# leggedrobotics/art_planner

Hardware: AMD Instinct MI355X
Metric: validated states/sec on 400x400@0.04m map (sample + validity check) (higher is better)
Workload: dtype f32; 1 GPU; C2: lazy_prm_star_min_update front end, 400x400@0.04m Perlin terrain (seed 1234) + 12 obstacles, YAML robot, batch sampler + validity checker; map=400x400@0.04, lanes=1

## Files before the change

art_planner_amd/context.py:

```python
from __future__ import annotations

import ctypes as C
from typing import Optional

import numpy as np

from . import _capi


def make_params(kind="yaml", **overrides) -> _capi.Params:
    L = _capi.load()
    p = _capi.Params()
    (L.artp_params_yaml if kind == "yaml" else L.artp_params_defaults)(C.byref(p))
    for k, v in overrides.items():
        setattr(p, k, v)
    return p


def _f32F(a) -> np.ndarray:
    return np.asfortranarray(a, dtype=np.float32)


class Context:

# ... 120 lines not shown

    def set_z_bounds(self, z_low, z_high):
        self._chk(self.L.artp_set_z_bounds(self.h, float(z_low), float(z_high)), "artp_set_z_bounds")
        self.z_bounds = (float(z_low), float(z_high))

    def set_r3_extent(self, max_extent):
        self._chk(self.L.artp_set_r3_extent(self.h, float(max_extent)), "artp_set_r3_extent")

    def check_motions_last_valid(self, s1, s2):
        s1 = np.ascontiguousarray(s1, np.float64).reshape(-1, 7)
        s2 = np.ascontiguousarray(s2, np.float64).reshape(-1, 7)
        n = s1.shape[0]
        valid = np.empty(n, np.uint8)
        t = np.empty(n, np.float64)
        st = np.empty((n, 7), np.float64)
        self._chk(self.L.artp_check_motions_last_valid(self.h, s1.ctypes.data, s2.ctypes.data, n, valid.ctypes.data,
                                                       t.ctypes.data, st.ctypes.data), "artp_check_motions_last_valid")
        return valid, t, st

    def sample_and_validate(self, seed, first_index, n, with_version=False):
        se3 = np.empty((n, 7), np.float64)
        valid = np.empty(n, np.uint8)
        ver = C.c_uint64(0)
        self._chk(self.L.artp_sample_and_validate(self.h, seed, first_index, n, se3.ctypes.data, valid.ctypes.data,
                                                  C.addressof(ver)), "artp_sample_and_validate")
        return (se3, valid, int(ver.value)) if with_version else (se3, valid)

    def map_version(self):
        return int(self.L.artp_map_version(self.h))

    def _reach_rect(self, rect):
        if rect is None:
            grid = getattr(self, "_grid", None)
            if grid is None:
                raise _capi.ArtpError("reachability: no map installed through this Context")
            return None, int(grid[0]), int(grid[1])
        r = np.ascontiguousarray(rect, np.int32).reshape(4)
        return r, max(int(r[2]), 0), max(int(r[3]), 0)

    def reachability_map(self, n_yaw=16, rect=None) -> np.ndarray:
        r, nr, nc = self._reach_rect(rect)
        out = np.zeros(nr * nc, np.uint32)
        self._chk(self.L.artp_reachability_map(self.h, int(n_yaw), r.ctypes.data if r is not None else None,
                                               out.ctypes.data), "artp_reachability_map")
        return out.reshape(nc, nr).T

    def reachability_map_dev(self, mask_t, n_yaw, rect=None):
        r, nr, nc = self._reach_rect(rect)
        if mask_t.numel() * mask_t.element_size() < nr * nc * 4:
            raise _capi.ArtpError("reachability_map_dev: mask_t holds fewer than nrows * ncols words")
        self._chk(self.L.artp_reachability_map_dev(self.h, int(n_yaw), r.ctypes.data if r is not None else None,
                                                   mask_t.data_ptr()), "artp_reachability_map_dev")

    def reachability_poses(self, n_yaw, rect=None) -> np.ndarray:
        r, nr, nc = self._reach_rect(rect)
        out = np.empty((nc, nr, max(int(n_yaw), 0), 7), np.float64)
        self._chk(self.L.artp_reachability_poses(self.h, int(n_yaw), r.ctypes.data if r is not None else None,
                                                 out.ctypes.data), "artp_reachability_poses")
        return out.transpose(1, 0, 2, 3)

    def reachability_halo(self) -> int:
        v = C.c_int(0)
        self._chk(self.L.artp_reachability_halo(self.h, C.byref(v)), "artp_reachability_halo")
        return v.value

    def cost_field(self, mask, n_yaw, sources, *, rect=None, reverse=False, objective=1, max_lon_vel=0.5,
                   max_lat_vel=0.1, max_ang_vel=0.5, plain_sweeps=False, inner_sweeps=64):
        from .field import CostField
        return CostField(self, mask, n_yaw, sources, rect=rect, reverse=reverse, objective=objective,
                         max_lon_vel=max_lon_vel, max_lat_vel=max_lat_vel, max_ang_vel=max_ang_vel,
                         plain_sweeps=plain_sweeps, inner_sweeps=inner_sweeps)

    def check_edges_interp(self, s1, s2):
        s1 = np.ascontiguousarray(s1, np.float64).reshape(-1, 7)
        s2 = np.ascontiguousarray(s2, np.float64).reshape(-1, 7)
        n = s1.shape[0]
        valid = np.empty(n, np.uint8)
        nint = np.empty(n, np.uint32)
        self._chk(self.L.artp_check_edges_interp(self.h, s1.ctypes.data, s2.ctypes.data, n,
                                                 valid.ctypes.data, nint.ctypes.data),
                  "artp_check_edges_interp")
        return valid, nint

    def use_torch_stream(self):
        import torch
        self._chk(self.L.artp_set_stream(self.h, C.c_void_p(torch.cuda.current_stream(self.device).cuda_stream)),
                  "artp_set_stream")

    def synchronize(self):
        self._chk(self.L.artp_synchronize(self.h), "artp_synchronize")

    def set_lane(self, lane: int):
        self._chk(self.L.artp_set_lane(self.h, int(lane)), "artp_set_lane")

    @property
    def lane(self) -> int:
        return int(self.L.artp_get_lane(self.h))

    def validate_states_dev(self, se3_t, valid_t, detail_t=None):
        n = se3_t.shape[0]
        self._chk(self.L.artp_validate_states_dev(self.h, se3_t.data_ptr(), n, valid_t.data_ptr(),
                                                  detail_t.data_ptr() if detail_t is not None else None),
                  "artp_validate_states_dev")

    def sample_states_dev(self, seed, first_index, n, out_t):
        self._chk(self.L.artp_sample_states_dev(self.h, seed, first_index, n, out_t.data_ptr()),
                  "artp_sample_states_dev")

    def sample_and_validate_dev(self, seed, first_index, n, se3_t, valid_t, count=False) -> Optional[int]:
        cnt = C.c_size_t(0)
        self._chk(self.L.artp_sample_and_validate_dev(self.h, seed, first_index, n, se3_t.data_ptr(),
                                                      valid_t.data_ptr(), C.byref(cnt) if count else None),
                  "artp_sample_and_validate_dev")
        return cnt.value if count else None

    def check_motions_dev(self, s1_t, s2_t, valid_t):
        self._chk(self.L.artp_check_motions_dev(self.h, s1_t.data_ptr(), s2_t.data_ptr(), s1_t.shape[0],
                                                valid_t.data_ptr()), "artp_check_motions_dev")

    def check_motions_last_valid_dev(self, s1_t, s2_t, valid_t, last_t_t, last_state_t=None):
        self._chk(self.L.artp_check_motions_last_valid_dev(self.h, s1_t.data_ptr(), s2_t.data_ptr(), s1_t.shape[0],
                                                           valid_t.data_ptr(), last_t_t.data_ptr(),
                                                           last_state_t.data_ptr() if last_state_t is not None else None),
                  "artp_check_motions_last_valid_dev")

    def check_edges_interp_dev(self, s1_t, s2_t, valid_t, nint_t=None):
        self._chk(self.L.artp_check_edges_interp_dev(self.h, s1_t.data_ptr(), s2_t.data_ptr(), s1_t.shape[0],
                                                     valid_t.data_ptr(),
                                                     nint_t.data_ptr() if nint_t is not None else None),
                  "artp_check_edges_interp_dev")

    def check_boxes_dev(self, slot, box, poses_t, hit_t, ec_t=None):
        box = np.ascontiguousarray(box, np.float32)
        self._chk(self.L.artp_check_boxes_dev(self.h, slot, box.ctypes.data, poses_t.data_ptr(),
                                              poses_t.shape[0], hit_t.data_ptr(),
                                              ec_t.data_ptr() if ec_t is not None else None),
                  "artp_check_boxes_dev")

    def compact_valid_dev(self, se3_t, valid_t, out_t, count_t):
        self._chk(self.L.artp_compact_valid_dev(self.h, se3_t.data_ptr(), valid_t.data_ptr(), se3_t.shape[0],
                                                out_t.data_ptr(), count_t.data_ptr()), "artp_compact_valid_dev")

    def algorithmic_vertices_dev(self, se3_t) -> int:
        v = C.c_uint64(0)
        self._chk(self.L.artp_algorithmic_vertices_dev(self.h, se3_t.data_ptr(), se3_t.shape[0], C.byref(v)),
                  "artp_algorithmic_vertices_dev")
        return v.value

    def pipeline_counters(self):
        out = (C.c_uint64 * 8)()
        self._chk(self.L.artp_debug_pipeline_counters(self.h, C.byref(out)), "artp_debug_pipeline_counters")
        return {"torso_queued": out[0], "feet_queued": out[4], "exact_grouping": out[1], "feet_plane_stage": out[5],
                "feet_partner_pass": out[6],
                "torso_staged_pass": out[2]}

    def partner_table(self, slot, shape):
        r = C.c_int(0)
        self._chk(self.L.artp_debug_partner_table(self.h, slot, None, 0, C.byref(r)), "artp_debug_partner_table")
        if r.value == 0:
            return None, 0
        out = np.empty(shape[0] * shape[1], np.uint8)
        self._chk(self.L.artp_debug_partner_table(self.h, slot, out.ctypes.data, out.size, C.byref(r)),
                  "artp_debug_partner_table")
        return out.reshape(shape[1], shape[0]), r.value

    def preprocess_map(self, elevation, len_x, len_y, pos_x=0.0, pos_y=0.0, traversability=None, kind="yaml",
                       observed=None, vertices=None, **overrides):
        p = _capi.PreprocessParams()
        (self.L.artp_preprocess_params_yaml if kind == "yaml" else self.L.artp_preprocess_params_defaults)(C.byref(p))
        for k, v in overrides.items():
            setattr(p, k, v)
        e = _f32F(elevation)
        t = _f32F(traversability) if traversability is not None else None
        o = _f32F(observed) if observed is not None else None
        vs = np.ascontiguousarray(vertices, np.float64).reshape(-1, 7) if vertices is not None else None
        inp = _capi.PreprocessInputs(e.ctypes.data, t.ctypes.data if t is not None else None,
                                     o.ctypes.data if o is not None else None,
                                     vs.ctypes.data if vs is not None else None, 0 if vs is None else vs.shape[0],
                                     e.shape[0], e.shape[1], len_x, len_y, pos_x, pos_y)
        h = C.c_void_p()
        self._chk(self.L.artp_preprocess_map_ex(self.h, C.byref(inp), C.byref(p), C.byref(h)), "artp_preprocess_map_ex")
        pm = PreprocessedMap(self, h, e.shape)
        pm.geom = (len_x, len_y, pos_x, pos_y)
        pm.params = p
        return pm

    def inpaint_layer(self, layer, mode=0):
        a = _f32F(layer)
        out = np.empty(a.shape, np.float32, order="F")
        n = C.c_uint64(0)
        self._chk(self.L.artp_inpaint_layer(self.h, a.ctypes.data, a.shape[0], a.shape[1], mode, out.ctypes.data,
                                            C.byref(n)), "artp_inpaint_layer")
        return out, n.value

    def cost_set_external_query(self, fn=None):
        if fn is None:
            self._ext_cost = None
            self._chk(self.L.artp_cost_set_external_query(self.h, _capi.COST_QUERY_FN(0), None), "artp_cost_set_external_query")
            return

        def thunk(_user, edges, b, cost):
            try:
                out = fn(np.ctypeslib.as_array(edges, shape=(b, 6)).copy())
                if out is None:
                    return 1
                np.ctypeslib.as_array(cost, shape=(b, 3))[:] = np.asarray(out, np.float32).reshape(b, 3)
                return 0
            except Exception:
                return 1

        self._ext_cost = _capi.COST_QUERY_FN(thunk)
        self._chk(self.L.artp_cost_set_external_query(self.h, self._ext_cost, None), "artp_cost_set_external_query")

    def cost_set_fc_path(self, mfma=True):
        self._chk(self.L.artp_cost_set_fc_path(self.h, 1 if mfma else 0), "artp_cost_set_fc_path")

    def cost_set_hole_filling(self, enabled=True):
        self._chk(self.L.artp_cost_set_hole_filling(self.h, 1 if enabled else 0), "artp_cost_set_hole_filling")

    def cost_load_weights(self, blob: bytes):
        buf = (C.c_char * len(blob)).from_buffer_copy(blob)
        self._chk(self.L.artp_cost_load_weights(self.h, buf, len(blob)), "artp_cost_load_weights")

    def cost_update_map(self, elev_xy, res, len_x, len_y, cx=0.0, cy=0.0):
        a = np.ascontiguousarray(elev_xy, np.float32)
        self._chk(self.L.artp_cost_update_map(self.h, a.ctypes.data, a.shape[0], a.shape[1], res, len_x, len_y,
                                              cx, cy), "artp_cost_update_map")

    def cost_update_map_dev(self, elev_xy_t, res, len_x, len_y, cx=0.0, cy=0.0):
        self._chk(self.L.artp_cost_update_map_dev(self.h, elev_xy_t.data_ptr(), elev_xy_t.shape[0], elev_xy_t.shape[1],
                                                  res, len_x, len_y, cx, cy), "artp_cost_update_map_dev")

    def cost_update_map_layer(self, layer, res, len_x, len_y, pos_x=0.0, pos_y=0.0):
        a = _f32F(layer)
        self._chk(self.L.artp_cost_update_map_layer(self.h, a.ctypes.data, a.shape[0], a.shape[1], res, len_x, len_y,
                                                    pos_x, pos_y), "artp_cost_update_map_layer")

    def cost_query(self, edges):
        e = np.ascontiguousarray(edges, np.float32).reshape(-1, 6)
        out = np.empty((e.shape[0], 3), np.float32)
        self._chk(self.L.artp_cost_query(self.h, e.ctypes.data, e.shape[0], out.ctypes.data), "artp_cost_query")
        return out

    def cost_query_cells(self, edges):
        e = np.ascontiguousarray(edges, np.float32).reshape(-1, 6)
        rows, cols = np.empty(e.shape[0], np.int32), np.empty(e.shape[0], np.int32)
        self._chk(self.L.artp_cost_debug_query_cells(self.h, e.ctypes.data, e.shape[0], rows.ctypes.data,
                                                     cols.ctypes.data), "artp_cost_debug_query_cells")
        return rows, cols

    def cost_debug_forms(self):
        out = (C.c_int32 * 4)()
        self._chk(self.L.artp_cost_debug_forms(self.h, out), "artp_cost_debug_forms")
        return dict(zip(("net", "c345_tile", "conv15_rows", "conv15_threads"), (int(v) for v in out)))

    def cost_fc_path(self):
        m, sc, d = C.c_int32(0), C.c_int32(0), C.c_float(0)
        self._chk(self.L.artp_cost_fc_path(self.h, C.byref(m), C.byref(sc), C.byref(d)), "artp_cost_fc_path")
        return {"mfma": int(m.value), "selfcheck": int(sc.value), "max_abs_diff": float(d.value)}

    def cost_query_dev(self, edges_t, cost_t):
        self._chk(self.L.artp_cost_query_dev(self.h, edges_t.data_ptr(), edges_t.shape[0], cost_t.data_ptr()),
                  "artp_cost_query_dev")

    def cost_feature_channels(self):
        ch = C.c_int(0)
        self._chk(self.L.artp_cost_feature_channels(self.h, C.byref(ch)), "artp_cost_feature_channels")
        return int(ch.value)

    def cost_features(self):
        ch = self.cost_feature_channels()
        fh, fw = C.c_int(0), C.c_int(0)
        self._chk(self.L.artp_cost_get_features_c(self.h, None, ch, C.byref(fh), C.byref(fw)), "artp_cost_get_features_c")
        out = np.empty((fh.value, fw.value, ch), np.float32)
        self._chk(self.L.artp_cost_get_features_c(self.h, out.ctypes.data, ch, C.byref(fh), C.byref(fw)),
                  "artp_cost_get_features_c")
        return out

    def compact_valid_indices_dev(self, valid_t, idx_t, count_t):
        self._chk(self.L.artp_compact_valid_indices_dev(self.h, valid_t.data_ptr(), valid_t.shape[0],
                                                        idx_t.data_ptr(), count_t.data_ptr()),
                  "artp_compact_valid_indices_dev")

    def pack_edge_results_dev(self, valid_t, ei_t, ej_t, cost_t, records_t, count_t):
        self._chk(self.L.artp_pack_edge_results_dev(self.h, valid_t.data_ptr(), ei_t.data_ptr(), ej_t.data_ptr(),
                                                    cost_t.data_ptr(), valid_t.shape[0], records_t.data_ptr(),
                                                    count_t.data_ptr()), "artp_pack_edge_results_dev")

    def pack_valid_bits_dev(self, valid_t, bits_t):
        self._chk(self.L.artp_pack_valid_bits_dev(self.h, valid_t.data_ptr(), valid_t.shape[0], bits_t.data_ptr()),
                  "artp_pack_valid_bits_dev")

    def indices_from_bits_dev(self, bits_t, n, idx_t, count_t):
        self._chk(self.L.artp_indices_from_bits_dev(self.h, bits_t.data_ptr(), n, idx_t.data_ptr(), count_t.data_ptr()),
                  "artp_indices_from_bits_dev")

    def materialise_from_bits_dev(self, seed, gathered_bits_t, prefix_bits, base_indices, cap, out_t, counts_t):
        n_ranks, words = gathered_bits_t.shape
        base = np.ascontiguousarray(base_indices, np.uint64)
        self._chk(self.L.artp_materialise_from_bits_dev(self.h, seed, gathered_bits_t.data_ptr(), n_ranks, words, prefix_bits,
                                                        base.ctypes.data, cap, out_t.data_ptr(), counts_t.data_ptr()),
                  "artp_materialise_from_bits_dev")

    def sample_states_at_dev(self, seed, base_index, idx_t, count_t, cap, out_t):
        self._chk(self.L.artp_sample_states_at_dev(self.h, seed, base_index, idx_t.data_ptr(), count_t.data_ptr(),
                                                   cap, out_t.data_ptr()), "artp_sample_states_at_dev")

# ... 44 lines not shown
```

art_planner_amd/csrc/artp_capi.hip:

```cpp
#include "../../include/artp_c.h"

#include <hip/hip_runtime.h>
#include <hipcub/hipcub.hpp>

#include <cmath>
#include <cstdio>
#include <atomic>
#include <chrono>
#include <cstdlib>
#include <cstring>
#include <mutex>
#include <string>
#include <array>
#include <vector>

#include "pipeline.h"
#include "cost_kernels.h"

using namespace artp;

#define ARTP_FEW_STATES 16
#define ARTP_SVC_MAX_STATES 2
#define FEW_EDGE_S1 0
#define FEW_EDGE_S2 (ARTP_FEW_EDGES * 7 * sizeof(double))
// ... 198 lines not shown
  }
  return ARTP_OK;
}

int publish_map_write(artp_ctx* c) {
  if (!c->map_written) HIP_TRY(c, hipEventCreateWithFlags(&c->map_written, hipEventDisableTiming));
  HIP_TRY(c, hipEventRecord(c->map_written, c->stream));
  c->map_seen[c->cur_lane] = ++c->map_write_seq;
  return ARTP_OK;
}

int lane_sees_map(artp_ctx* c) {
  if (c->map_seen[c->cur_lane] != c->map_write_seq && c->map_written) {
    HIP_TRY(c, hipStreamWaitEvent(c->stream, c->map_written, 0));
    c->map_seen[c->cur_lane] = c->map_write_seq;
  }
  return ARTP_OK;
}

void fill_robot(artp_ctx* c) {
  const artp_params& p = c->params;
  RobotDev& r = c->robot;
  r.torso[0] = (float)p.torso_length;
  r.torso[1] = (float)p.torso_width;
  r.torso[2] = (float)p.torso_height;
  r.foot[0] = (float)p.reach_x;
  r.foot[1] = (float)p.reach_y;
  r.foot[2] = (float)p.reach_z;
  r.torso_off[0] = (float)p.torso_off_x;
  r.torso_off[1] = (float)p.torso_off_y;
  r.torso_off[2] = (float)(p.torso_off_z - p.feet_off_z);
  r.feet_off_x = (float)p.feet_off_x;
  r.feet_off_y = (float)p.feet_off_y;
  r.unknown_space_untraversable = p.unknown_space_untraversable;
  r.reach_z = p.reach_z;
  r.max_pitch_pert = p.max_pitch_pert;
  r.max_roll_pert = p.max_roll_pert;
}

void r_from_2_axes(float* R, float ax, float ay, float az, float bx, float by, float bz) {
  float l = sqrtf(ax * ax + ay * ay + az * az);
  if (l <= 0.0f) return;
  l = 1.0f / l;
  ax *= l; ay *= l; az *= l;
  const float k = ax * bx + ay * by + az * bz;
  bx -= k * ax; by -= k * ay; bz -= k * az;
  l = sqrtf(bx * bx + by * by + bz * bz);
  if (l <= 0.0f) return;
  l = 1.0f / l;
  bx *= l; by *= l; bz *= l;
  R[0] = ax; R[4] = ay; R[8] = az;
  R[1] = bx; R[5] = by; R[9] = bz;
  R[2] = -by * az + ay * bz;
  R[6] = -bz * ax + az * bx;
  R[10] = -bx * ay + ax * by;
  R[3] = R[7] = R[11] = 0.0f;
}

int size_scratch(artp_ctx* c) {
  const artp_params& p = c->params;
  const double d_torso = std::sqrt(p.torso_length * p.torso_length + p.torso_width * p.torso_width +
                                   p.torso_height * p.torso_height);
  const double d_foot = std::sqrt(p.reach_x * p.reach_x + p.reach_y * p.reach_y + p.reach_z * p.reach_z);
  double diag = d_torso > d_foot ? d_torso : d_foot;
  double spacing = 1e30;
  int max_n = 2;
  for (int s = 0; s < 2; ++s) {
    if (!c->have_field[s]) continue;
    spacing = std::fmin(spacing, (double)std::fmin(c->field[s].sample_w, c->field[s].sample_d));
    max_n = std::max(max_n, std::max(c->field[s].nW, c->field[s].nD));
  }
  if (spacing > 1e29) return ARTP_OK;
  int maxdim = (int)std::ceil(diag / spacing) + 4;
  if (maxdim > max_n) maxdim = max_n;
  if (maxdim < 4) maxdim = 4;
  long verts = (long)maxdim * maxdim;
  long tris = 2L * (maxdim - 1) * (maxdim - 1);
  if (tris > 4096) tris = 4096;
  verts = (verts + 3) & ~3L;
  tris = (tris + 7) & ~7L;
  long tab = 64;
  while (tab < 2 * tris && tab < 4096) tab <<= 1;
  if (maxdim > 64) {
    c->last_error = "box window wider than 64 samples: not supported by the packed triangle ids";
    return ARTP_ERR_CAPACITY;
  }
  c->caps_full = ScratchCaps{64 * 36, (int)verts, (int)tris, (int)tab};
  c->caps_scan = ScratchCaps{64 * 36, (int)verts, (int)(tris < 1024 ? tris : 1024), 0};
  {
    int fdim = (int)std::ceil(d_foot / spacing) + 4;
    if (fdim > max_n) fdim = max_n;
    if (fdim < 4) fdim = 4;
    long fv = ((long)fdim * fdim + 3) & ~3L;
    long ft = (2L * (fdim - 1) * (fdim - 1) + 7) & ~7L;
    if (ft > 1024) ft = 1024;
    c->caps_feet = ScratchCaps{32 * 36, (int)fv, (int)ft, 0};
    c->caps_feet_wave = ScratchCaps{64 * 36, (int)fv, (int)ft, 0};
    long ftf = (2L * (fdim - 1) * (fdim - 1) + 7) & ~7L;
    if (ftf > 4096) ftf = 4096;
    long ftab = 64;
    while (ftab < 2 * ftf && ftab < 4096) ftab <<= 1;
    c->caps_foot_full = ScratchCaps{64 * 36, (int)fv, (int)ftf, (int)ftab};
  }
  if (scratch_bytes_per_wave(c->caps_full) > 160 * 1024 ||
      scratch_bytes_per_wave(c->caps_scan) * ARTP_WAVES_PER_BLOCK > 160 * 1024 ||
      scratch_bytes_per_wave(c->caps_full) + 4 * scratch_bytes_per_wave(c->caps_foot_full) > 160 * 1024) {
    c->last_error = "box too large for the LDS window tile";
    return ARTP_ERR_CAPACITY;
  }
  return ARTP_OK;
}

size_t lds_full(const artp_ctx* c) { return scratch_bytes_per_wave(c->caps_full); }
size_t lds_scan(const artp_ctx* c) { return scratch_bytes_per_wave(c->caps_scan) * ARTP_WAVES_PER_BLOCK; }
size_t lds_feet(const artp_ctx* c) { return scratch_bytes_per_wave(c->caps_feet) * 4 * ARTP_WAVES_PER_BLOCK; }
size_t lds_feet_wave(const artp_ctx* c) { return scratch_bytes_per_wave(c->caps_feet_wave) * ARTP_WAVES_PER_BLOCK; }
size_t lds_few(const artp_ctx* c) {
  return scratch_bytes_per_wave(c->caps_full) + 4 * scratch_bytes_per_wave(c->caps_foot_full);
}

int opt_in_lds(artp_ctx* c, const void* fn, size_t bytes) {
  static std::mutex mu;
  static std::vector<std::pair<std::pair<int, const void*>, int>> set;
  std::lock_guard<std::mutex> lock(mu);
  int* have = nullptr;
  for (auto& e : set)
    if (e.first.first == c->device && e.first.second == fn) have = &e.second;
  if (have && *have >= (int)bytes) return ARTP_OK;
  HIP_TRY(c, hipFuncSetAttribute(fn, hipFuncAttributeMaxDynamicSharedMemorySize, (int)bytes));
  if (have)
    *have = (int)bytes;
  else
    set.push_back({{c->device, fn}, (int)bytes});
  return ARTP_OK;
}

#define ARTP_OPT_IN(c, kernel, bytes)                                                       \
  do {                                                                                      \
    const int _rc = opt_in_lds((c), reinterpret_cast<const void*>(kernel), (bytes));        \
    if (_rc != ARTP_OK) return _rc;                                                         \
  } while (0)

int set_kernel_lds(artp_ctx* c) {
  ARTP_OPT_IN(c, check_boxes_kernel<1>, lds_full(c));
  ARTP_OPT_IN(c, validate_states_kernel<1>, lds_full(c));
  ARTP_OPT_IN(c, plane_stage_kernel<1>, lds_full(c));
  ARTP_OPT_IN(c, validate_few_kernel, lds_few(c));
  ARTP_OPT_IN(c, check_motions_few_kernel, lds_few(c));
  ARTP_OPT_IN(c, validate_service_kernel, lds_few(c));
  ARTP_OPT_IN(c, check_motions_pool_kernel, lds_few(c));
  ARTP_OPT_IN(c, (resolve_boxes_kernel<ARTP_WAVES_PER_BLOCK, 64, 3>), lds_scan(c));
  ARTP_OPT_IN(c, (resolve_boxes_kernel<ARTP_WAVES_PER_BLOCK, 16, 1>), lds_feet(c));
  ARTP_OPT_IN(c, (resolve_boxes_kernel<ARTP_WAVES_PER_BLOCK, 64, 2>), lds_feet_wave(c));
  return ARTP_OK;
}

int grid_full(const artp_ctx* c, size_t tasks) {
  size_t per_cu = (160 * 1024) / (lds_full(c) ? lds_full(c) : 1);
  if (per_cu > 16) per_cu = 16;
  if (per_cu < 1) per_cu = 1;
  size_t g = (size_t)c->n_cus * per_cu;
  if (tasks && tasks < g) g = tasks;
  return (int)(g ? g : 1);
}
int grid_scan(const artp_ctx* c, size_t lds) {
  size_t per_cu = (160 * 1024) / (lds ? lds : 1);
  if (per_cu > 8) per_cu = 8;
  if (per_cu < 1) per_cu = 1;
  return (int)((size_t)c->n_cus * per_cu);
}

unsigned grid_sub(const artp_ctx* c, int per_cu) {
  const unsigned g = (unsigned)c->n_cus * (unsigned)per_cu;
  return (g + ARTP_NSUB - 1) / ARTP_NSUB * ARTP_NSUB;
}

int partner_radius(const artp_ctx* c, int slot) {
  const FieldDev& f = c->field[slot];
  const float* side = slot == 1 ? c->robot.foot : c->robot.torso;
  const double diag = std::sqrt((double)side[0] * side[0] + (double)side[1] * side[1] + (double)side[2] * side[2]);
  const int R = (int)std::ceil(diag / std::fmin((double)f.sample_w, (double)f.sample_d)) + 3;
  return R > 63 ? -1 : R;
}

static void partner_rect_extent(const FieldDev& f, const PartnerRects& pr, int margin, int* max_cells, int* max_rows) {
  *max_cells = *max_rows = 1;
  for (int k = 0; k < pr.n; ++k) {
    const int nx = std::min(pr.x1[k] + margin, f.nW - 1) - std::max(pr.x0[k] - margin, 0) + 1;
    const int nz = std::min(pr.z1[k] + margin, f.nD - 1) - std::max(pr.z0[k] - margin, 0) + 1;
    *max_cells = std::max(*max_cells, nx * nz);
    *max_rows = std::max(*max_rows, pr.z1[k] - pr.z0[k] + 1);
  }
}

int build_partner_table_full(artp_ctx* c, int slot) {
  FieldDev& f = c->field[slot];
  f.partner_flags = nullptr;
  f.partner_R = 0;
  c->partner_R_built[slot] = -1;
  const int R = partner_radius(c, slot);
  if (R < 0) return ARTP_OK;
  PartnerRects all{};
  all.n = 1;
  all.x0[0] = all.z0[0] = 0;
  all.x1[0] = f.nW - 1;
  all.z1[0] = f.nD - 1;
  const int ncell = f.nW * f.nD;
  hipLaunchKernelGGL(tri_raw_rects_kernel, dim3((ncell + 255) / 256, 1), dim3(256), 0, c->stream, f, all,
                     c->tri_raw_buf[slot], c->partner_cnt[slot]);
  hipLaunchKernelGGL(partner_count_kernel<false>, dim3((ncell + 255) / 256, 2 * R + 1, 1), dim3(256), 0, c->stream, f, R,
                     (const float4*)c->tri_raw_buf[slot], c->partner_cnt[slot], all, 1);
  hipLaunchKernelGGL(partner_flags_from_counts_kernel, dim3((ncell + 255) / 256, 1), dim3(256), 0, c->stream, f.nW, f.nD, all,
                     0, (const unsigned*)c->partner_cnt[slot], c->partner_buf[slot]);
  HIP_TRY(c, hipGetLastError());
  c->partner_R_built[slot] = R;
  f.partner_flags = c->partner_buf[slot];
  f.partner_R = R;
  return ARTP_OK;
}

int partner_update_begin(artp_ctx* c, int slot, const int* dirty, int n_dirty, PartnerRects* pr) {
  const FieldDev& f = c->field[slot];
  *pr = PartnerRects{};
  const int R = partner_radius(c, slot);
  if (R < 0 || c->partner_R_built[slot] != R || n_dirty <= 0) return ARTP_OK;
  std::vector<std::array<int, 4>> rects;
  for (int k = 0; k < n_dirty; ++k)
    rects.push_back({std::max(dirty[4 * k] - 1, 0), std::max(dirty[4 * k + 1] - 1, 0), std::min(dirty[4 * k + 2], f.nW - 2),
                     std::min(dirty[4 * k + 3], f.nD - 2)});
  for (bool merged = true; merged;) {
    merged = false;
    for (size_t a = 0; a < rects.size() && !merged; ++a)
      for (size_t b = a + 1; b < rects.size() && !merged; ++b)
        if (rects[a][0] <= rects[b][2] && rects[b][0] <= rects[a][2] && rects[a][1] <= rects[b][3] && rects[b][1] <= rects[a][3]) {
          rects[a] = {std::min(rects[a][0], rects[b][0]), std::min(rects[a][1], rects[b][1]),
                      std::max(rects[a][2], rects[b][2]), std::max(rects[a][3], rects[b][3])};
          rects.erase(rects.begin() + b);
          merged = true;
        }
  }
  if (rects.size() > 8) return ARTP_OK;
  size_t changed = 0;
  for (const auto& r : rects) changed += (size_t)(r[2] - r[0] + 1) * (r[3] - r[1] + 1);
  if (changed * 4 > (size_t)f.nW * f.nD) return ARTP_OK;
  for (size_t k = 0; k < rects.size(); ++k) {
    if (rects[k][2] < rects[k][0] || rects[k][3] < rects[k][1]) continue;
    const int j = pr->n++;
    pr->x0[j] = rects[k][0]; pr->z0[j] = rects[k][1]; pr->x1[j] = rects[k][2]; pr->z1[j] = rects[k][3];
  }
  if (pr->n == 0) return ARTP_OK;
  int cells, rows;
  partner_rect_extent(f, *pr, R, &cells, &rows);
  hipLaunchKernelGGL(partner_count_kernel<true>, dim3((cells + 255) / 256, rows, pr->n), dim3(256), 0, c->stream, f, R,
                     (const float4*)c->tri_raw_buf[slot], c->partner_cnt[slot], *pr, -1);
  HIP_TRY(c, hipGetLastError());
  c->partner_R_built[slot] = -1;
  c->tables[slot].valid = 0;
  c->field[slot].partner_flags = nullptr;
  c->field[slot].partner_R = 0;
  return ARTP_OK;
}

int partner_update_end(artp_ctx* c, int slot, const PartnerRects& pr) {
  if (pr.n == 0) return build_partner_table_full(c, slot);
  FieldDev& f = c->field[slot];
  const int R = partner_radius(c, slot);
  int cells0, cellsR, rows;
  partner_rect_extent(f, pr, 0, &cells0, &rows);
  partner_rect_extent(f, pr, R, &cellsR, &rows);
  hipLaunchKernelGGL(tri_raw_rects_kernel, dim3((cells0 + 255) / 256, pr.n), dim3(256), 0, c->stream, f, pr,
                     c->tri_raw_buf[slot], c->partner_cnt[slot]);
  hipLaunchKernelGGL(partner_count_kernel<true>, dim3((cellsR + 255) / 256, rows, pr.n), dim3(256), 0, c->stream, f, R,
                     (const float4*)c->tri_raw_buf[slot], c->partner_cnt[slot], pr, 1);
  hipLaunchKernelGGL(partner_count_kernel<false>, dim3((cells0 + 255) / 256, 2 * R + 1, pr.n), dim3(256), 0, c->stream, f, R,
                     (const float4*)c->tri_raw_buf[slot], c->partner_cnt[slot], pr, 1);
  hipLaunchKernelGGL(partner_flags_from_counts_kernel, dim3((cellsR + 255) / 256, pr.n), dim3(256), 0, c->stream, f.nW, f.nD,
                     pr, R, (const unsigned*)c->partner_cnt[slot], c->partner_buf[slot]);
  HIP_TRY(c, hipGetLastError());
  c->partner_R_built[slot] = R;
  f.partner_flags = c->partner_buf[slot];
  f.partner_R = R;
  return ARTP_OK;
}

int build_tables(artp_ctx* c, int slot, const PartnerRects* pr = nullptr) {
  const FieldDev& f = c->field[slot];
  const size_t elems = (size_t)f.nW * f.nD;
  if (c->table_elems[slot] < elems) {
    if (c->table_buf[slot]) HIP_TRY(c, hipFree(c->table_buf[slot]));
    if (c->flag_buf[slot]) HIP_TRY(c, hipFree(c->flag_buf[slot]));
    if (c->stride_buf[slot]) HIP_TRY(c, hipFree(c->stride_buf[slot]));
    c->stride_buf[slot] = nullptr;
    if (c->partner_buf[slot]) HIP_TRY(c, hipFree(c->partner_buf[slot]));
    if (c->partner_cnt[slot]) HIP_TRY(c, hipFree(c->partner_cnt[slot]));
    c->partner_cnt[slot] = nullptr;
    HIP_TRY(c, hipMalloc(reinterpret_cast<void**>(&c->partner_cnt[slot]), elems * sizeof(unsigned)));
    if (c->tri_raw_buf[slot]) HIP_TRY(c, hipFree(c->tri_raw_buf[slot]));
    c->tri_raw_buf[slot] = nullptr;
    HIP_TRY(c, hipMalloc(reinterpret_cast<void**>(&c->tri_raw_buf[slot]), elems * sizeof(float4)));
    c->table_buf[slot] = nullptr;
    c->flag_buf[slot] = nullptr;
    c->partner_buf[slot] = nullptr;
    HIP_TRY(c, hipMalloc(reinterpret_cast<void**>(&c->partner_buf[slot]), (elems + 3) / 4 * 4));
    c->partner_R_built[slot] = -1;
    HIP_TRY(c, hipMalloc(reinterpret_cast<void**>(&c->table_buf[slot]), 12 * elems * sizeof(float)));
    HIP_TRY(c, hipMalloc(reinterpret_cast<void**>(&c->flag_buf[slot]), 6 * elems));
    HIP_TRY(c, hipMalloc(reinterpret_cast<void**>(&c->stride_buf[slot]), (elems / 2 + 3 * (f.nW + f.nD) + 16) * sizeof(unsigned)));
    c->table_elems[slot] = elems;
  }
  float2* mm[6];
  unsigned char* fl[6];
  for (int l = 0; l < 6; ++l) {
    mm[l] = reinterpret_cast<float2*>(c->table_buf[slot]) + (size_t)l * elems;
    fl[l] = reinterpret_cast<unsigned char*>(c->flag_buf[slot]) + (size_t)l * elems;
  }
  const int n = (int)elems;
  hipLaunchKernelGGL(table_level0_kernel, dim3((n + 255) / 256), dim3(256), 0, c->stream, f.data, n, mm[0], fl[0]);
  for (int l = 1; l < 6; ++l)
    hipLaunchKernelGGL(table_level_up_kernel, dim3((n + 255) / 256), dim3(256), 0, c->stream,
                       (const float2*)mm[l - 1], (const unsigned char*)fl[l - 1], f.nW, f.nD, 1 << (l - 1), mm[l],
                       fl[l]);
  HIP_TRY(c, hipGetLastError());
  TablesDev& t = c->tables[slot];
  t.mm = mm[2];
  t.fl = fl[2];
  t.stride = (unsigned)elems;
  t.has_nan = f.has_nan;
  t.has_nonfinite = c->layer_has_nonfinite[slot];
  {
    unsigned off[ARTP_STRIDE_LEVELS + 1] = {0};
    for (int l = 0; l < ARTP_STRIDE_LEVELS; ++l) {
      const int s = 2 << l;
      off[l + 1] = off[l] + (unsigned)(((f.nW + s - 1) / s) * ((f.nD + s - 1) / s));
    }
    t.st = c->stride_buf[slot];
    t.st_off1 = off[1];
    t.st_off2 = off[2];
    hipLaunchKernelGGL(stride_tables_kernel, dim3((off[3] + 255) / 256), dim3(256), 0, c->stream, t.mm, t.fl, t.stride,
                       f.nW, f.nD, off[1], off[2], off[3], c->stride_buf[slot]);
    HIP_TRY(c, hipGetLastError());
  }
  const int rc_partner = pr ? partner_update_end(c, slot, *pr) : build_partner_table_full(c, slot);
  if (rc_partner != ARTP_OK) return rc_partner;
  t.valid = 1;
  return ARTP_OK;
}

int ensure_recs(artp_ctx* c, size_t n) { return ensure_tmp(c, 7, n * sizeof(PoseRec)); }

int launch_validate_pipeline(artp_ctx* c, const double* se3, size_t n, uint8_t* valid, bool recs_ready = false) {
  if (n >= (1ull << 32)) {
    c->last_error = "batch too large (state index is 32 bit)";
    return ARTP_ERR_INVALID_ARG;
  }
  int rc = ensure_recs(c, n);
  if (rc) return rc;
  PoseRec* recs = static_cast<PoseRec*>(c->tmp[7]);
  if (!recs_ready)
    hipLaunchKernelGGL(pose_rec_kernel, dim3((unsigned)((n + 255) / 256)), dim3(256), 0, c->stream, c->field[0], se3, n,
                       recs);
  const size_t per_block_states = 64 * ARTP_CLASSIFY_SUB;
  const size_t n_blocks = (n + per_block_states - 1) / per_block_states;
  const size_t seg_t = ((n_blocks + ARTP_NSUB - 1) / ARTP_NSUB) * per_block_states;
  rc = ensure_tmp(c, 4, 5 * ARTP_NSUB * seg_t * sizeof(PendingBox));
  if (rc) return rc;
  const size_t ctr_bytes = 128 + (size_t)2 * ARTP_NSUB * 128;
  rc = ensure_tmp(c, 5, ctr_bytes + ((5 + 4 + 4) * n + 5 * (size_t)ARTP_NSUB * seg_t) * sizeof(unsigned) + 64);
  if (rc) return rc;
  PipelineQueues q;
  q.q1 = static_cast<PendingBox*>(c->tmp[4]);
  q.counters = static_cast<unsigned long long*>(c->tmp[5]);
  q.sub = q.counters + 16;
  q.seg_t = seg_t;
  q.q2 = reinterpret_cast<unsigned*>(static_cast<char*>(c->tmp[5]) + ctr_bytes);
  q.q3 = q.q2 + 5 * n;
  q.q5 = q.q3 + 4 * n;
  q.q4 = q.q5 + 4 * n;
  q.q6 = q.q4 + 4 * (size_t)ARTP_NSUB * seg_t;
  q.feet_base = (unsigned long long)ARTP_NSUB * seg_t;
  HIP_TRY(c, hipMemsetAsync(q.counters, 0, ctr_bytes, c->stream));
  const size_t per_block = 64 * ARTP_CLASSIFY_SUB;
  hipLaunchKernelGGL(classify_states_kernel, dim3((unsigned)((n + per_block - 1) / per_block)),
                     dim3(ARTP_CLASSIFY_THREADS), 0, c->stream,
                     c->field[0], c->field[1], c->tables[0], c->tables[1], c->geom, c->robot, (const PoseRec*)recs, n,
                     valid, q);
#ifdef ARTP_VARIANTS
  if (c->feet_dense)
    hipLaunchKernelGGL(feet_stream2_kernel<ARTP_STREAM_WAVES>, dim3(grid_sub(c, ARTP_FEET_WAVES_PER_SIMD)), dim3(64 * ARTP_STREAM_WAVES), 0,
                       c->stream, c->field[1], c->robot, q, valid);
  else
#endif
    hipLaunchKernelGGL(feet_stream_kernel<ARTP_STREAM_WAVES>, dim3(grid_sub(c, ARTP_FEET_WAVES_PER_SIMD)), dim3(64 * ARTP_STREAM_WAVES), 0,
                       c->stream, c->field[1], c->robot, q, valid);
  hipLaunchKernelGGL(feet_lane_kernel, dim3((unsigned)c->n_cus * 8), dim3(ARTP_LANE_THREADS), 0, c->stream,
                     c->field[1], c->robot, q, valid);
  {
    const ScratchCaps caps_stream{0, 0, 0, 0};
    const size_t lds_stream = 0;
    hipLaunchKernelGGL((resolve_boxes_kernel<ARTP_WAVES_PER_BLOCK, 64, 0>), dim3(grid_sub(c, ARTP_TORSO_WGS_PER_CU)),
                       dim3(64 * ARTP_WAVES_PER_BLOCK), lds_stream, c->stream, c->field[0], c->robot, q, valid,
                       caps_stream, c->d_error, c->tables[0].valid ? c->tables[0].mm : (const float2*)nullptr);
  }
  hipLaunchKernelGGL((resolve_boxes_kernel<ARTP_WAVES_PER_BLOCK, 64, 3>), dim3(grid_scan(c, lds_scan(c))),
                     dim3(64 * ARTP_WAVES_PER_BLOCK), lds_scan(c), c->stream, c->field[0], c->robot, q, valid,
                     c->caps_scan, c->d_error);
  hipLaunchKernelGGL((resolve_boxes_kernel<ARTP_WAVES_PER_BLOCK, 16, 1>), dim3(grid_scan(c, lds_feet(c))),
                     dim3(64 * ARTP_WAVES_PER_BLOCK), lds_feet(c), c->stream, c->field[1], c->robot, q, valid,
                     c->caps_feet, c->d_error);
  hipLaunchKernelGGL((resolve_boxes_kernel<ARTP_WAVES_PER_BLOCK, 64, 2>), dim3(grid_scan(c, lds_feet_wave(c))),
                     dim3(64 * ARTP_WAVES_PER_BLOCK), lds_feet_wave(c), c->stream, c->field[1], c->robot, q, valid,
                     c->caps_feet_wave, c->d_error);
  hipLaunchKernelGGL(plane_stage_kernel<1>, dim3(grid_full(c, 0)), dim3(64), lds_full(c), c->stream,
                     c->field[0], c->field[1], c->robot, q, valid, c->caps_full, c->d_error);
  HIP_TRY(c, hipGetLastError());
  return ARTP_OK;
}

int check_error_flag(artp_ctx* c) {
  int flag = 0;
  HIP_TRY(c, hipMemcpyAsync(&flag, c->d_error, sizeof(int), hipMemcpyDeviceToHost, c->stream));
  HIP_TRY(c, hipStreamSynchronize(c->stream));
  if (flag) {
    HIP_TRY(c, hipMemsetAsync(c->d_error, 0, sizeof(int), c->stream));
    c->last_error = "a box window exceeded the LDS tile capacity";
    return ARTP_ERR_CAPACITY;
  }
  return ARTP_OK;
}

}

extern "C" {

void artp_params_defaults(artp_params* p) {
  p->torso_length = 1.05; p->torso_width = 0.55; p->torso_height = 0.2;
  p->torso_off_x = 0.0; p->torso_off_y = 0.0; p->torso_off_z = 0.0;
  p->feet_off_x = 0.362; p->feet_off_y = 0.225; p->feet_off_z = -0.525;
  p->reach_x = 0.25; p->reach_y = 0.1; p->reach_z = 0.15;
  p->unknown_space_untraversable = 1;
  p->max_pitch_pert = 10.0 / 180 * M_PI;
  p->max_roll_pert = 3.33 / 180 * M_PI;
  p->sample_from_distribution = 1;
}

void artp_params_yaml(artp_params* p) {
  p->torso_length = 1.31; p->torso_width = 0.65; p->torso_height = 0.3;
  p->torso_off_x = 0.0; p->torso_off_y = 0.0; p->torso_off_z = 0.04;
  p->feet_off_x = 0.51; p->feet_off_y = 0.2; p->feet_off_z = -0.475;
  p->reach_x = 0.2; p->reach_y = 0.2; p->reach_z = 0.2;
  p->unknown_space_untraversable = 1;
  p->max_pitch_pert = 10 * M_PI / 180;
  p->max_roll_pert = 3.33 * M_PI / 180;
  p->sample_from_distribution = 1;
}

const char* artp_status_string(int s) {
  switch (s) {
    case ARTP_OK: return "ok";
    case ARTP_ERR_INVALID_ARG: return "invalid argument";
    case ARTP_ERR_NO_DEVICE: return "no usable HIP device (this library has no CPU fallback)";
    case ARTP_ERR_HIP: return "HIP runtime error";
    case ARTP_ERR_NO_MAP: return "required layer not uploaded";
    case ARTP_ERR_CAPACITY: return "box window exceeds the LDS tile capacity";
    case ARTP_ERR_NO_WEIGHTS: return "motion-cost weights not loaded";
    case ARTP_ERR_TIMEOUT: return "timed out waiting for a device group";
    case ARTP_ERR_COMM: return "RCCL unavailable or a communicator call failed";
    case ARTP_ERR_COST_FUNC: return "Motion cost call failed";
    default: return "unknown status";
  }
}

const char* artp_last_error(const artp_ctx* ctx) { return ctx ? ctx->last_error.c_str() : ""; }
const char* artp_device_arch(const artp_ctx* ctx) { return ctx ? ctx->arch.c_str() : ""; }

static void pool_stop(artp_ctx* c);
static void svc_stop(artp_ctx* c) {
  if (!c->svc || !c->svc_launched) return;
  c->svc->n_quit = 0x100u;
  std::atomic_thread_fence(std::memory_order_seq_cst);
  const auto t0 = std::chrono::steady_clock::now();
  while (c->svc->running && std::chrono::steady_clock::now() - t0 < std::chrono::milliseconds(200))
    ;
  (void)hipStreamSynchronize(c->svc_stream);
  c->svc_launched = false;
}

static int svc_start(artp_ctx* c) {
  if (!c->svc) {
    void *p = nullptr, *pd = nullptr;
    HIP_TRY(c, hipHostMalloc(&p, sizeof(SvcMailbox), hipHostMallocMapped));
    HIP_TRY(c, hipHostGetDevicePointer(&pd, p, 0));
    std::memset(p, 0, sizeof(SvcMailbox));
    c->svc = static_cast<SvcMailbox*>(p);
    c->svc_dev = static_cast<SvcMailbox*>(pd);
    HIP_TRY(c, hipStreamCreateWithFlags(&c->svc_stream, hipStreamNonBlocking));
    HIP_TRY(c, hipEventCreateWithFlags(&c->svc_after_map, hipEventDisableTiming));
  }
  HIP_TRY(c, hipEventRecord(c->svc_after_map, c->stream));
  HIP_TRY(c, hipStreamWaitEvent(c->svc_stream, c->svc_after_map, 0));
  c->svc->n_quit = 0u;
  c->svc->running = 1u;
  c->svc->resp = c->svc_seq << 8;
  c->svc->req_seq = c->svc_seq;
  std::atomic_thread_fence(std::memory_order_seq_cst);
  hipLaunchKernelGGL(validate_service_kernel, dim3(1), dim3(320), lds_few(c), c->svc_stream, c->field[0], c->field[1], c->geom,
                     c->robot, c->svc_dev, c->svc_seq, c->caps_full, c->caps_foot_full);
  HIP_TRY(c, hipGetLastError());
  c->svc_launched = true;
  c->svc_map_version = c->map_version.load(std::memory_order_acquire);
  ++c->svc_launches;
  return ARTP_OK;
}

static int svc_validate(artp_ctx* c, const double* se3, size_t n, uint8_t* valid) {
  for (int attempt = 0; attempt < 3; ++attempt) {
    const bool stale = c->svc_launched && c->svc_map_version != c->map_version.load(std::memory_order_acquire);
    if (stale) svc_stop(c);
    if (c->svc_launched && !c->svc->running) {
      (void)hipStreamSynchronize(c->svc_stream);
      c->svc_launched = false;
    }
    if (!c->svc_launched) {
      const int rc = svc_start(c);
      if (rc) return rc;
    }
    if (n > 1) std::memcpy(c->svc->state1, se3 + 7, 7 * sizeof(double));
    std::memcpy(c->svc->state0, se3, 7 * sizeof(double));
    c->svc->n_quit = (uint32_t)n;
    std::atomic_thread_fence(std::memory_order_seq_cst);
    const uint32_t seq = ++c->svc_seq;
    c->svc->req_seq = seq;
    std::atomic_thread_fence(std::memory_order_seq_cst);
    const auto t0 = std::chrono::steady_clock::now();
    bool answered = false, gone = false;
    for (unsigned spin = 0;; ++spin) {
      if ((c->svc->resp >> 8) == (seq & 0xffffffu)) { answered = true; break; }
      if ((spin & 255u) == 255u) {
        if (!c->svc->running) { gone = true; break; }
        if (std::chrono::steady_clock::now() - t0 > std::chrono::milliseconds(50)) break;
      }
    }
    if (!answered && gone && (c->svc->resp >> 8) == (seq & 0xffffffu)) answered = true;
    if (answered) {
      const uint32_t r = c->svc->resp;
      bool overflow = false;
      for (size_t i = 0; i < n; ++i) {
        const unsigned b = (r >> (2 * i)) & 3u;
        valid[i] = b & 1u;
        overflow = overflow || (b & 2u);
      }
      ++c->svc_requests;
      if (overflow) {
        c->last_error = "a box window exceeded the LDS tile capacity";
        return ARTP_ERR_CAPACITY;
      }
      return ARTP_OK;
    }
    if (gone) {
      (void)hipStreamSynchronize(c->svc_stream);
      c->svc_launched = false;
      --c->svc_seq;
      continue;
    }
    c->last_error = "the persistent latency service did not answer within 50 ms";
    svc_stop(c);
    return ARTP_ERR_TIMEOUT;
// ... 2689 lines not shown
```

art_planner_amd/csrc/pipeline.h:

```cpp
#pragma once

#include <hip/hip_fp16.h>

#include "kernels.h"

namespace artp {

#define ARTP_TABLE_LEVELS 4

struct TablesDev {
  const float2* mm;
  const unsigned char* fl;
  unsigned stride;
  int has_nan;
  int has_nonfinite;
  int valid;
  const unsigned* st;
  unsigned st_off1, st_off2;
};

#define ARTP_STRIDE_LEVELS 3

__global__ void __launch_bounds__(256)
table_level0_kernel(const float* __restrict__ data, int n, float2* __restrict__ mm, unsigned char* __restrict__ fl) {
// ... 871 lines not shown
#endif

template <int WAVES, int G, int PASS>
__global__ void __launch_bounds__(64 * WAVES)
resolve_boxes_kernel(FieldDev fld, RobotDev rb, PipelineQueues q, uint8_t* __restrict__ valid,
                     ScratchCaps caps, int* __restrict__ error_flag, const float2* __restrict__ mm4 = nullptr) {
  extern __shared__ __attribute__((aligned(16))) char smem[];
  constexpr int GPW = 64 / G;
  const int lane = threadIdx.x & 63;
  const int gl = lane & (G - 1);
  const int unit_in_block = (threadIdx.x >> 6) * GPW + (lane / G);
  const WaveScratch s = carve_scratch(smem, unit_in_block, caps);
  const bool direct = PASS == 1 && fwd_total(q, 1) < ARTP_LANE_SCAN_MIN;
  const bool feet = (PASS == 1 && !direct) || PASS == 2;
  const int sq = blockIdx.x % ARTP_NSUB;
  const unsigned long long count =
      PASS == 0 ? *sub_counter(q, 0, sq)
                : (PASS == 3 ? fwd_total(q, 0) : (direct ? fwd_total(q, 1) : q.counters[PASS == 1 ? 5 : 6]));
  const unsigned long long first = PASS == 0 ? sub_base(q, 0, sq) : 0ull;
  const unsigned long long nblk = PASS == 0 ? gridDim.x / ARTP_NSUB : gridDim.x;
  const unsigned long long blk = PASS == 0 ? blockIdx.x / ARTP_NSUB : blockIdx.x;
  const unsigned long long stride = nblk * WAVES * GPW;
#ifdef ARTP_STAGE_TIMING
  unsigned long long t_acc[8] = {0, 0, 0, 0, 0, 0, 0, 0};
  const long long t_begin = clock64();
#endif
  unsigned long long next = PASS == 0 ? 0ull : blk * WAVES * GPW + unit_in_block, chunk_end = 0ull;
  __shared__ unsigned fwd_slots[PASS == 0 ? WAVES : 1][ARTP_TORSO_CHUNK];
  unsigned* fs = fwd_slots[PASS == 0 ? (threadIdx.x >> 6) : 0];
  if (PASS == 0 && lane < ARTP_TORSO_CHUNK) fs[lane] = 0u;
  unsigned long long chunk_first = 0ull;
  for (;;) {
    if constexpr (PASS == 0) {
      if (next >= chunk_end) {
        fwd_flush_slots<ARTP_TORSO_CHUNK>(fs, sub_fwd(q, 0, sq), q.q6 + fwd_base(q, 0, sq), lane);
        unsigned long long c0 = 0;
        if (lane == 0) c0 = atomicAdd(sub_cursor(q, 0, sq), (unsigned long long)ARTP_TORSO_CHUNK);
        c0 = __shfl(c0, 0);
        if (c0 >= count) break;
        next = c0;
        chunk_first = c0;
        chunk_end = c0 + ARTP_TORSO_CHUNK < count ? c0 + ARTP_TORSO_CHUNK : count;
      }
    } else {
      if (next >= count) break;
    }
    const unsigned long long it = next;
    next += PASS == 0 ? 1ull : stride;
    const unsigned long long item =
        PASS == 0 ? first + it
                  : (unsigned long long)(PASS == 1 ? (direct ? fwd_item(q, 1, q.q4, it) : q.q3[it])
                                                   : (PASS == 2 ? q.q5[it] : fwd_item(q, 0, q.q6, it)));
#ifdef ARTP_STAGE_TIMING
    long long t_prev = clock64();
#endif
    const PendingBox rec = q.q1[item];
    if (valid[rec.state] == 0) continue;
    BoxHF b;
    box_from_record(rec, rb, b);
    ARTP_T_MARK(0);
    int result = 0, ec, fast_r = 2;
    bool decided = false;
    if constexpr (PASS == 0) {
      if (fld.partner_flags != nullptr && (rec.kind & ARTP_REC_ALL_FINITE)) {
        __shared__ unsigned short hot_blocks[WAVES][ARTP_HOT_BLOCKS];
        if (wave_vertex_stream_blocks<ARTP_TORSO_U>(fld, mm4, b, hot_blocks[threadIdx.x >> 6], lane)) {
          result = 1;
          decided = true;
        } else {
          ARTP_T_MARK(2);
          const int r = grp_corner_stage_direct<G>(fld, b, lane);
          if (r != 2) {
            result = r;
            decided = true;
          }
        }
        ARTP_T_MARK(4);
      }
      if (!decided) {
        if (gl == 0) fs[it - chunk_first] = (unsigned)item + 1u;
      } else if (gl == 0 && result != 0) {
        valid[rec.state] = 0;
      }
      continue;
    }
    const int total = (b.maxX - b.minX + 1) * (b.maxZ - b.minZ + 1);
    if (total > s.cap_verts) {
      if (gl == 0) atomicExch(error_flag, 1);
      continue;
    }
    WindowStats w;
    if (!decided) {
      grp_scan_window<G>(fld, b, s, lane, w);
      ARTP_T_MARK(1);
      decided = !feet && decide_exits(b, w, result, ec);
    }
    if (!decided) {
      const bool vhit = !feet && grp_vertex_pass<G>(fld, b, s, lane, w.allFinite);
      ARTP_T_MARK(2);
      if (vhit) {
        result = 1;
        decided = true;
      } else if (PASS == 1) {
        const int r = grp_plane_stage_corners<G>(fld, b, s, lane, 0, true);
        ARTP_T_MARK(4);
        if (r != 2) {
          result = r;
          decided = true;
        } else if (gl == 0) {
          const unsigned long long slot = atomicAdd(&q.counters[6], 1ull);
          q.q5[slot] = (unsigned)item;
        }
      } else if (PASS == 3 && fld.partner_flags != nullptr &&
                 (fast_r = grp_plane_stage_corners<G>(fld, b, s, lane, 0, true)) != 2) {
        ARTP_T_MARK(4);
        result = fast_r;
        decided = true;
      } else {
        const int T = grp_compact_triangles<G, true>(b, s, lane);
        ARTP_T_MARK(3);
#ifdef ARTP_STAGE_TIMING
        const int r = (T == 0) ? 0 : (T < 0 ? 2 : grp_plane_stage_corners<G>(fld, b, s, lane, T, false, t_acc));
#else
        const int r = (T == 0) ? 0 : (T < 0 ? 2 : grp_plane_stage_corners<G>(fld, b, s, lane, T));
#endif
        ARTP_T_MARK(4);
        if (r != 2) {
          result = r;
          decided = true;
        } else if (gl == 0) {
          const unsigned long long slot = atomicAdd(&q.counters[1], 1ull);
          q.q2[slot] = (unsigned)item;
        }
      }
    }
    if (decided && gl == 0) {
      const bool ok = (rec.kind & 1u) ? (result != 0) : (result == 0);
      if (!ok) valid[rec.state] = 0;
    }
    wave_lds_sync();
  }
#ifdef ARTP_STAGE_TIMING
  if (gl == 0) {
    for (int k = 0; k < 8; ++k) atomicAdd(&g_stage_cycles[G == 64 ? 0 : 1][k], t_acc[k]);
    atomicAdd(&g_stage_cycles[G == 64 ? 0 : 1][8], (unsigned long long)(clock64() - t_begin));
    atomicAdd(&g_stage_cycles[G == 64 ? 0 : 1][9], 1ull);
  }
#endif
}

template <int WAVES>
__global__ void __launch_bounds__(64 * WAVES)
plane_stage_kernel(FieldDev fb, FieldDev ff, RobotDev rb, PipelineQueues q, uint8_t* __restrict__ valid,
                   ScratchCaps caps, int* __restrict__ error_flag) {
  extern __shared__ __attribute__((aligned(16))) char smem[];
  const int lane = threadIdx.x & 63;
  const WaveScratch s = carve_scratch(smem, threadIdx.x >> 6, caps);
  const unsigned long long count = q.counters[1];
  const unsigned long long stride = (unsigned long long)gridDim.x * WAVES;
  for (unsigned long long item = (unsigned long long)blockIdx.x * WAVES + (threadIdx.x >> 6); item < count;
       item += stride) {
    const PendingBox rec = q.q1[q.q2[item]];
    if (valid[rec.state] == 0) continue;
    BoxHF b;
    box_from_record(rec, rb, b);
    const bool foot = (rec.kind & 1u) != 0;
    WindowStats w;
    if (foot)
      wave_scan_window(ff, b, s, lane, w);
    else
      wave_scan_window(fb, b, s, lane, w);
    const int T = wave_compact_triangles<true>(b, s, lane);
    int result;
    if (T < 0)
      result = (foot ? wave_plane_stage_unlisted(ff, b, s, lane) : wave_plane_stage_unlisted(fb, b, s, lane)) ? 1 : 0;
    else
      result = (T > 0 && (foot ? wave_plane_stage(ff, b, s, lane, T) : wave_plane_stage(fb, b, s, lane, T))) ? 1 : 0;
    if (lane == 0) {
      const bool ok = (rec.kind & 1u) ? (result != 0) : (result == 0);
      if (!ok) valid[rec.state] = 0;
    }
    wave_lds_sync();
  }
}

#ifdef ARTP_VARIANTS
#include "pipeline_variants.h"
#endif

}
```

Before: 3.659 billion states/s.

## Fuse torso scan and feet wave resolve launches into one tail kernel

Replaces the separate torso-scan and feet-wave resolve_boxes launches with a single tail_boxes_kernel. It walks the torso forward queue and the feet partner queue in one grid, and for grouped boxes with small triangle counts it solves the plane stage in place using a table carved from the candidate scratch. Only boxes that overflow are pushed to a new queue slot, and plane_stage_kernel now reads its count from that slot. This removes one launch, merges the load-balancing tails of the two kernels, and shrinks the serial plane-stage work, at the cost of running feet boxes with torso-sized LDS occupancy and adding some divergence.

```diff
diff --git a/art_planner_amd/context.py b/art_planner_amd/context.py
--- a/art_planner_amd/context.py
+++ b/art_planner_amd/context.py
@@ -296,7 +296,7 @@
         self._chk(self.L.artp_debug_pipeline_counters(self.h, C.byref(out)), "artp_debug_pipeline_counters")
         return {"torso_queued": out[0], "feet_queued": out[4], "exact_grouping": out[1], "feet_plane_stage": out[5],
                 "feet_partner_pass": out[6],
-                "torso_staged_pass": out[2]}
+                "torso_staged_pass": out[2], "tail_overflow": out[3]}
 
     def partner_table(self, slot, shape):
         r = C.c_int(0)
diff --git a/art_planner_amd/csrc/artp_capi.hip b/art_planner_amd/csrc/artp_capi.hip
--- a/art_planner_amd/csrc/artp_capi.hip
+++ b/art_planner_amd/csrc/artp_capi.hip
@@ -374,6 +374,7 @@
   ARTP_OPT_IN(c, (resolve_boxes_kernel<ARTP_WAVES_PER_BLOCK, 64, 3>), lds_scan(c));
   ARTP_OPT_IN(c, (resolve_boxes_kernel<ARTP_WAVES_PER_BLOCK, 16, 1>), lds_feet(c));
   ARTP_OPT_IN(c, (resolve_boxes_kernel<ARTP_WAVES_PER_BLOCK, 64, 2>), lds_feet_wave(c));
+  ARTP_OPT_IN(c, tail_boxes_kernel<ARTP_WAVES_PER_BLOCK>, lds_scan(c));
   return ARTP_OK;
 }
 
@@ -623,17 +624,14 @@
                        dim3(64 * ARTP_WAVES_PER_BLOCK), lds_stream, c->stream, c->field[0], c->robot, q, valid,
                        caps_stream, c->d_error, c->tables[0].valid ? c->tables[0].mm : (const float2*)nullptr);
   }
-  hipLaunchKernelGGL((resolve_boxes_kernel<ARTP_WAVES_PER_BLOCK, 64, 3>), dim3(grid_scan(c, lds_scan(c))),
-                     dim3(64 * ARTP_WAVES_PER_BLOCK), lds_scan(c), c->stream, c->field[0], c->robot, q, valid,
-                     c->caps_scan, c->d_error);
   hipLaunchKernelGGL((resolve_boxes_kernel<ARTP_WAVES_PER_BLOCK, 16, 1>), dim3(grid_scan(c, lds_feet(c))),
                      dim3(64 * ARTP_WAVES_PER_BLOCK), lds_feet(c), c->stream, c->field[1], c->robot, q, valid,
                      c->caps_feet, c->d_error);
-  hipLaunchKernelGGL((resolve_boxes_kernel<ARTP_WAVES_PER_BLOCK, 64, 2>), dim3(grid_scan(c, lds_feet_wave(c))),
-                     dim3(64 * ARTP_WAVES_PER_BLOCK), lds_feet_wave(c), c->stream, c->field[1], c->robot, q, valid,
-                     c->caps_feet_wave, c->d_error);
+  hipLaunchKernelGGL(tail_boxes_kernel<ARTP_WAVES_PER_BLOCK>, dim3(grid_scan(c, lds_scan(c))),
+                     dim3(64 * ARTP_WAVES_PER_BLOCK), lds_scan(c), c->stream, c->field[0], c->field[1], c->robot, q, valid,
+                     c->caps_scan, c->caps_feet_wave.verts, c->caps_feet_wave.tris, c->d_error);
   hipLaunchKernelGGL(plane_stage_kernel<1>, dim3(grid_full(c, 0)), dim3(64), lds_full(c), c->stream,
-                     c->field[0], c->field[1], c->robot, q, valid, c->caps_full, c->d_error);
+                     c->field[0], c->field[1], c->robot, q, valid, c->caps_full, c->d_error, 3);
   HIP_TRY(c, hipGetLastError());
   return ARTP_OK;
 }
diff --git a/art_planner_amd/csrc/pipeline.h b/art_planner_amd/csrc/pipeline.h
--- a/art_planner_amd/csrc/pipeline.h
+++ b/art_planner_amd/csrc/pipeline.h
@@ -1047,11 +1047,11 @@
 template <int WAVES>
 __global__ void __launch_bounds__(64 * WAVES)
 plane_stage_kernel(FieldDev fb, FieldDev ff, RobotDev rb, PipelineQueues q, uint8_t* __restrict__ valid,
-                   ScratchCaps caps, int* __restrict__ error_flag) {
+                   ScratchCaps caps, int* __restrict__ error_flag, int count_slot = 1) {
   extern __shared__ __attribute__((aligned(16))) char smem[];
   const int lane = threadIdx.x & 63;
   const WaveScratch s = carve_scratch(smem, threadIdx.x >> 6, caps);
-  const unsigned long long count = q.counters[1];
+  const unsigned long long count = q.counters[count_slot];
   const unsigned long long stride = (unsigned long long)gridDim.x * WAVES;
   for (unsigned long long item = (unsigned long long)blockIdx.x * WAVES + (threadIdx.x >> 6); item < count;
        item += stride) {
@@ -1079,6 +1079,79 @@
   }
 }
 
+#define ARTP_TAIL_TAB 512
+template <bool FOOT>
+__device__ __forceinline__ int tail_one_box(const FieldDev& fld, const BoxHF& b, const WaveScratch& s, int lane,
+                                            bool tab_fits, bool& grouped) {
+  constexpr int G = 64;
+  grouped = false;
+  const int total = (b.maxX - b.minX + 1) * (b.maxZ - b.minZ + 1);
+  if (total > s.cap_verts) return -1;
+  WindowStats w;
+  grp_scan_window<G>(fld, b, s, lane, w);
+  int T;
+  if (!FOOT) {
+    int result = 0, ec;
+    if (decide_exits(b, w, result, ec)) return result;
+    if (grp_vertex_pass<G>(fld, b, s, lane, w.allFinite)) return 1;
+    if (fld.partner_flags != nullptr) {
+      const int fast_r = grp_plane_stage_corners<G>(fld, b, s, lane, 0, true);
+      if (fast_r != 2) return fast_r;
+    }
+  }
+  T = grp_compact_triangles<G, true>(b, s, lane);
+  const int r = (T == 0) ? 0 : (T < 0 ? 2 : grp_plane_stage_corners<G>(fld, b, s, lane, T));
+  if (r != 2) return r;
+  grouped = true;
+  if (T < 0 || 2 * T > ARTP_TAIL_TAB || !tab_fits) return 2;
+  WaveScratch sg = s;
+  sg.tab = reinterpret_cast<unsigned*>(s.cand);
+  sg.tab_size = ARTP_TAIL_TAB;
+  wave_lds_sync();
+  return wave_plane_stage(fld, b, sg, lane, T) ? 1 : 0;
+}
+
+template <int WAVES>
+__global__ void __launch_bounds__(64 * WAVES)
+tail_boxes_kernel(FieldDev fb, FieldDev ff, RobotDev rb, PipelineQueues q, uint8_t* __restrict__ valid,
+                  ScratchCaps caps, int foot_verts, int foot_tris, int* __restrict__ error_flag) {
+  extern __shared__ __attribute__((aligned(16))) char smem[];
+  const int lane = threadIdx.x & 63;
+  const int wave = __builtin_amdgcn_readfirstlane((int)(threadIdx.x >> 6));
+  const WaveScratch s_torso = carve_scratch(smem, wave, caps);
+  WaveScratch s_foot = s_torso;
+  s_foot.cap_verts = foot_verts;
+  s_foot.cap_tris = foot_tris;
+  const bool tab_fits = caps.cand >= ARTP_TAIL_TAB * (int)sizeof(unsigned);
+  const unsigned long long n6 = fwd_total(q, 0), count = n6 + q.counters[6];
+  const unsigned long long stride = (unsigned long long)gridDim.x * WAVES;
+  for (unsigned long long it = (unsigned long long)blockIdx.x * WAVES + wave; it < count; it += stride) {
+    const bool foot = it >= n6;
+    const unsigned item = foot ? q.q5[it - n6] : fwd_item(q, 0, q.q6, it);
+    const PendingBox rec = q.q1[item];
+    if (valid[rec.state] == 0) continue;
+    BoxHF b;
+    box_from_record(rec, rb, b);
+    bool grouped;
+    const int result = foot ? tail_one_box<true>(ff, b, s_foot, lane, tab_fits, grouped)
+                            : tail_one_box<false>(fb, b, s_torso, lane, tab_fits, grouped);
+    if (lane == 0) {
+      if (result < 0) {
+        atomicExch(error_flag, 1);
+      } else {
+        if (grouped) atomicAdd(&q.counters[1], 1ull);
+        if (result == 2) {
+          q.q2[atomicAdd(&q.counters[3], 1ull)] = item;
+        } else {
+          const bool ok = foot ? (result != 0) : (result == 0);
+          if (!ok) valid[rec.state] = 0;
+        }
+      }
+    }
+    wave_lds_sync();
+  }
+}
+
 #ifdef ARTP_VARIANTS
 #include "pipeline_variants.h"
 #endif
```

Result: no change. 3.677 billion states/s, median of 6 (+0.5%).
